# deeplearning-wisc/MCM

Measured on AMD Instinct MI355X. Metric: images/sec MCM-scored (CLIP-B/16, 1000 prompts), higher is better.
Workload: dtype fp16; 1 GPU; MCM scoring, CLIP-ViT-B/16 (12L vision tower, random-init weights), K=1000 prompts pre-encoded, batch 512/GPU, fp32 NCHW pixels resident in HBM -> [B] scores; batch_per_gpu=512, prompts=1000, parallelism=image-sharded x1

## Files before the change

include/mcm.h:

```cpp
#ifndef MCM_H_
#define MCM_H_

#include <stdint.h>

#ifdef __cplusplus
extern "C" {
#endif

#define MCM_ABI_VERSION 5

#define MCM_OK 0
#define MCM_EINVAL (-1)
#define MCM_ENOMEM (-2)
#define MCM_EHIP (-3)
#define MCM_ENOWEIGHT (-4)
#define MCM_ENAME (-5)
#define MCM_ESHAPE (-6)
#define MCM_ERANGE (-7)

#define MCM_PREC_BF16 0
#define MCM_PREC_F32 1
#define MCM_PREC_F16 2

#define MCM_DT_F32 0
// ... 203 lines not shown
int mcm_debug_attention_variant(int32_t variant);
int mcm_debug_attn_spin_budget(int64_t polls);
int mcm_debug_clear_faults(mcm_handle* h);
int mcm_debug_op_attention(mcm_handle* h, int32_t prec, const void* qkv_dev, void* out_dev, int32_t nseq, int32_t seq_len,
                           int32_t heads, int32_t causal, int32_t qrows, int32_t reverse, void* stream);
int mcm_debug_op_attention_split(mcm_handle* h, const void* qkv_dev, void* out_dev, int32_t nseq, int32_t seq_len,
                                 int32_t heads, int32_t qrows, int32_t reverse, void* stream);
int mcm_debug_op_attention_hd(mcm_handle* h, int32_t prec, const void* qkv_dev, void* out_dev, int32_t nseq, int32_t seq_len,
                              int32_t heads, int32_t head_dim, int32_t causal, int32_t qrows, int32_t reverse, void* stream);
int mcm_debug_op_attention_split_hd(mcm_handle* h, const void* qkv_dev, void* out_dev, int32_t nseq, int32_t seq_len,
                                    int32_t heads, int32_t head_dim, int32_t qrows, int32_t reverse, void* stream);
int mcm_debug_vision_front(mcm_handle* h, const void* pixels_dev, int32_t pixel_format, int32_t x2, int32_t B, int32_t stage,
                           int32_t poison, float* resid_out_dev, void* ln_out_dev, void* stream);
int mcm_debug_op_pool_project(mcm_handle* h, const float* x_dev, int64_t x_rows, const int32_t* row_idx_host, int32_t row_stride,
                              int32_t n, int32_t D, const float* gamma_dev, const float* beta_dev, float eps,
                              const float* proj_dev, int32_t P, float* out_dev, int32_t normalize, void* stream);
int mcm_debug_op_text_embed(mcm_handle* h, const int32_t* ids_host, int32_t vocab, const float* tok_dev, const float* pos_dev,
                            float* x_dev, int32_t K, int32_t S, int32_t D, void* stream);
int mcm_debug_gemm_dbg(int32_t bits);
int mcm_debug_qkv_chunks(int32_t n);
int mcm_debug_nsplit(int32_t n);
int mcm_debug_gemm_group_n(int32_t gn);
int mcm_debug_patch_fold(int32_t on);
int mcm_debug_resize_fused_only(int32_t on);
int mcm_debug_persistent_grid(int32_t n);
int mcm_debug_ln_fold(int32_t on);
int mcm_debug_qkv_head_major(int32_t on);
int mcm_debug_ln_tail(int32_t on);
int mcm_debug_ln_cluster(int32_t on);
int mcm_debug_ln_cluster_spin(int32_t polls);
int mcm_debug_ln_row(int32_t on);
int mcm_debug_ln_cluster_deferred(mcm_handle* h, uint64_t* count_host);
int mcm_debug_ln_tail_timeouts(mcm_handle* h, uint64_t* count_host);
#endif

#ifdef __cplusplus
}
#endif
#endif
```

mcm_amd/csrc/attention.hip:

```cpp
#include "common.hpp"

namespace {

__device__ __forceinline__ int ktile_off(int r, int c) {
  const int p = r >> 1;
  return p * 256 + ((((r & 1) << 3) | ((c ^ p) & 7)) << 4);
}

#ifdef MCM_HARNESS
__host__ __device__ constexpr int vt_stride(int LP) {
  return ((LP * 2 - 16 + 255) / 256) * 256 + 16;
}

template <int PREC, int LP, bool CAUSAL>
__global__ __launch_bounds__(256, 2) void attn_bf16_kernel(const uint16_t* __restrict__ qkv,
                                                           uint16_t* __restrict__ out, int L,
                                                           int heads, int qrows, int rev) {
  enter_precision_mode<PREC>();
  extern __shared__ __attribute__((aligned(16))) char smem[];
  constexpr int NT = LP / 16;
  constexpr int NU = LP / 32;
  constexpr int VS = vt_stride(LP);
  constexpr int MAXQB = (LP / 16 + 3) / 4;
  char* Ks = smem;
// ... 1537 lines not shown
  const int nt = (L + 15) / 16;
#ifdef MCM_HARNESS
  if (g_attn_variant == 10 && nseq % 8 == 0) rev |= 2;
  if (g_attn_variant == 11) rev |= 4;
#endif
  bool persistent = nt == 13 && !causal && !hm && qrows == L && (int64_t)nseq * heads >= 16 * (int64_t)device_cu_count();
#ifdef MCM_HARNESS
  if (g_attn_variant == 36) persistent = false;
  if (g_attn_variant == 21) persistent = nt == 13 && !causal && !hm;
#endif
  if (persistent) return launch_ps<PREC, 13, 12, 4>(qkv, out, nseq, L, heads, qrows, s, rev, fault);
#define MCM_TR_EXACT(N, W, O) \
  if (nt == N && !causal) return launch_tr<PREC, N, W, O, false, N - 1>(qkv, out, nseq, L, heads, false, qrows, s, rev, hm)
  MCM_TR_EXACT(4, 4, 3); MCM_TR_EXACT(13, 8, 3); MCM_TR_EXACT(17, 8, 3);
#undef MCM_TR_EXACT
#define MCM_TR(N, W, O) \
  if (nt <= N) return launch_tr<PREC, N, W, O>(qkv, out, nseq, L, heads, causal, qrows, s, rev, hm)
  MCM_TR(1, 4, 3); MCM_TR(2, 4, 3); MCM_TR(3, 4, 3); MCM_TR(4, 4, 3); MCM_TR(5, 4, 3); MCM_TR(6, 4, 3);
  MCM_TR(8, 4, 3); MCM_TR(10, 8, 3); MCM_TR(13, 8, 3); MCM_TR(17, 8, 3); MCM_TR(18, 8, 3);
#undef MCM_TR
  return hipErrorInvalidValue;
}


}

#ifdef MCM_HARNESS
void attention_set_variant(int v) { g_attn_variant = v; }
void attention_set_spin_budget(unsigned int polls) { g_ps_spin_budget = polls; }
#endif

hipError_t launch_attention(int prec, const void* qkv, void* out, int nseq, int L, int heads, int head_dim,
                            bool causal, int qrows, hipStream_t s, bool reverse, int hm, bool split, unsigned int* fault) {
  if (nseq <= 0 || L <= 0 || heads <= 0) return hipErrorInvalidValue;
  if (head_dim != 64 && head_dim != H80) return hipErrorInvalidValue;
  if (qrows <= 0 || qrows > L) qrows = L;
  if (head_dim == H80) {
    if (causal || hm || L > LONG_MAX_L) return hipErrorInvalidValue;
    const int rv = reverse ? 1 : 0;
    if (split) {
      if (prec != MCM_PREC_F16 || (heads * H80) % 64) return hipErrorInvalidValue;
      return launch_hd80<MCM_PREC_F16, true>(qkv, out, nseq, L, heads, qrows, s, rv);
    }
    if (prec == MCM_PREC_F16) return launch_hd80<MCM_PREC_F16, false>(qkv, out, nseq, L, heads, qrows, s, rv);
    if (prec == MCM_PREC_BF16) return launch_hd80<MCM_PREC_BF16, false>(qkv, out, nseq, L, heads, qrows, s, rv);
    if (prec == MCM_PREC_F32) return launch_hd80<MCM_PREC_F32, false>(qkv, out, nseq, L, heads, qrows, s, rv);
    return hipErrorInvalidValue;
// ... 76 lines not shown
```

mcm_amd/csrc/common.hpp:

```cpp
#pragma once
#include <hip/hip_runtime.h>
#include <stdint.h>

#include "../../include/mcm.h"

struct PerDeviceFlag {
  bool done[64] = {};
  static int dev() { int d = 0; return hipGetDevice(&d) == hipSuccess && d >= 0 && d < 64 ? d : -1; }
  bool get() const { const int d = dev(); return d >= 0 && done[d]; }
  void set() { const int d = dev(); if (d >= 0) done[d] = true; }
};

inline int device_cu_count() {
  static int cus[64] = {};
  int dev = 0;
  if (hipGetDevice(&dev) != hipSuccess || dev < 0) return 0;
  if (dev < 64 && cus[dev] > 0) return cus[dev];
  int n = 0;
  if (hipDeviceGetAttribute(&n, hipDeviceAttributeMultiprocessorCount, dev) != hipSuccess) return 0;
  if (dev < 64) cus[dev] = n;
  return n;
}

typedef __attribute__((ext_vector_type(8))) __bf16 bf16x8_t;
// ... 230 lines not shown
hipError_t launch_gemm_row64_ln(int prec, const GemmArgs& a, hipStream_t s, int stages);
hipError_t launch_row64_block_w(const void* w, void* blocked, int N, int K, hipStream_t s);
void gemm_set_group_n(int gn);
void gemm_set_dbg(int d);
void gemm_set_variant(int v);
void attention_set_variant(int v);
void attention_set_spin_budget(unsigned int polls);
#endif

hipError_t launch_layernorm(int prec, const float* x, const float* g, const float* b, void* y,
                            int M, int D, float eps, bool out_f32, hipStream_t s,
                            size_t x_stride = 0, size_t y_stride = 0, bool reverse = false,
                            unsigned int* sat = nullptr, bool split = false);

hipError_t launch_layernorm_pre(int prec, float* x, const float* g0, const float* b0, const float* g1,
                                const float* b1, void* y, int M, int D, float eps, hipStream_t s,
                                bool reverse = false, unsigned int* sat = nullptr, const float* cls = nullptr,
                                const float* pos0 = nullptr, int ntok = 0, bool split = false);

hipError_t launch_attention(int prec, const void* qkv, void* out, int nseq, int L, int heads, int head_dim,
                            bool causal, int qrows, hipStream_t s, bool reverse = false, int hm = 0, bool split = false,
                            unsigned int* fault = nullptr);

hipError_t launch_patchify(int prec, const float* pixels, void* patches, int B, int image,
                           int patch, int kpad, hipStream_t s, bool split = false);
hipError_t launch_patchify_u8(int prec, const uint8_t* pixels, void* patches, int B, int image,
                              int patch, int kpad, const float* mean, const float* stdv,
                              hipStream_t s, bool split = false);
hipError_t launch_bank_reduce(const float* feats, int K, int T, int P, float* bank, hipStream_t s);
hipError_t launch_text_embed(const int32_t* ids, const float* tok, const float* pos, float* x,
                             int K, int S, int D, hipStream_t s);
hipError_t launch_cvt_weight(int prec, const float* src, void* dst, int rows, int cols,
                             int cols_pad, hipStream_t s);
hipError_t launch_cvt_weight_split(int prec, const float* src, void* dst, int rows, int cols,
                                   int cols_pad, hipStream_t s);
hipError_t launch_count_inexact(int prec, const float* src, size_t n, unsigned long long* count, hipStream_t s);

hipError_t launch_pool_project(const float* x, const int32_t* row_idx, int row_stride, int n,
                               int D, const float* g, const float* b, float eps,
                               const float* proj, int P, float* out, hipStream_t s,
                               bool normalize = true);
hipError_t launch_maha_prepare(const float* means, const float* prec, int C, int P, double* w, double* c,
                               hipStream_t s);
hipError_t launch_maha_score(const float* feats, int B, const float* prec, const double* w, const double* c,
                             int C, int P, float* scores, hipStream_t s);
hipError_t launch_maha_fit(const float* feats, int B, int P, const float* shift, double* gram, double* sum,
// ... 44 lines not shown
```

mcm_amd/csrc/embed.hip:

```cpp
#include "common.hpp"

namespace {

template <int OUT, bool X2 = false>
__global__ __launch_bounds__(256) void patchify_kernel(const float* __restrict__ px, void* out,
                                                       int B, int S, int P, int kpad) {
  const int g = S / P, np = g * g, kreal = 3 * P * P;
  const size_t total = (size_t)B * np * kpad;
  for (size_t i = (size_t)blockIdx.x * 256 + threadIdx.x; i < total;
       i += (size_t)gridDim.x * 256) {
    const int k = (int)(i % kpad);
    const size_t m = i / kpad;
    float v = 0.f;
    if (k < kreal) {
      const int b = (int)(m / np), p = (int)(m % np);
      const int gy = p / g, gx = p % g;
      const int c = k / (P * P), rem = k % (P * P), py = rem / P, pxx = rem % P;
      v = px[(((size_t)b * 3 + c) * S + gy * P + py) * S + gx * P + pxx];
    }
    if constexpr (X2) {
      const _Float16 hi = (_Float16)v;
      _Float16* dst = (_Float16*)out + m * 2 * kpad + split_col(k);
      dst[0] = hi;
      dst[64] = (_Float16)(v - (float)hi);
// ... 172 lines not shown
  for (int i = 0; i < NWP; ++i) tot += red[i];
  const float mean = tot / (float)D;
  const float c = tid < D ? xv - mean : 0.f;
  float cw = 0.f;
  float q;
  if constexpr (WIDE) {
    if (t2 < D) cw = xw - mean;
    q = wave_sum(fmaf(cw, cw, c * c));
  } else {
    q = wave_sum(c * c);
  }
  if (lane == 0) red[NWP + wave] = q;
  __syncthreads();
  tot = 0.f;
#pragma unroll
  for (int i = 0; i < NWP; ++i) tot += red[NWP + i];
  const float rstd = 1.0f / sqrtf(tot / (float)D + eps);
  if (tid < D) y[tid] = c * rstd * g[tid] + b[tid];
  if constexpr (WIDE) {
    if (t2 < D) y[t2] = cw * rstd * g[t2] + b[t2];
  }
  __syncthreads();
  float sq = 0.f;
  for (int p = wave; p < P; p += NWP) {
    const float* w = proj + (size_t)p * D;
    float a = 0.f;
    for (int d = lane * 4; d < D; d += 256) {
      const float4 wv = *(const float4*)(w + d);
      a = fmaf(wv.x, y[d], a);
      a = fmaf(wv.y, y[d + 1], a);
      a = fmaf(wv.z, y[d + 2], a);
      a = fmaf(wv.w, y[d + 3], a);
    }
    a = wave_sum(a);
    if (lane == 0) {
      o[p] = a;
      sq += a * a;
    }
  }
  __syncthreads();
  if (lane == 0) red[wave] = sq;
  __syncthreads();
  tot = 0.f;
#pragma unroll
  for (int i = 0; i < NWP; ++i) tot += red[i];
  const float rn = normalize ? 1.0f / sqrtf(tot) : 1.0f;
  for (int p = tid; p < P; p += NWP * 64) out[(size_t)n * P + p] = o[p] * rn;
}

inline int grid_for(size_t total) {
  size_t g = (total + 255) / 256;
  return (int)(g > 4096 ? 4096 : (g ? g : 1));
}

}

hipError_t launch_patchify(int prec, const float* pixels, void* patches, int B, int image,
                           int patch, int kpad, hipStream_t s, bool split) {
  const int g = image / patch;
  if (split) {
// ... 93 lines not shown
```

mcm_amd/csrc/mcm_api.hip:

```cpp
#include <algorithm>
#include <map>
#include <string>
#include <vector>

#include <math.h>
#include <stdlib.h>
#include <string.h>

#include "common.hpp"

namespace {

thread_local std::string g_create_err;

struct Param {
  std::vector<int64_t> shape;
  int64_t numel = 0;
  float* dev = nullptr;
  bool set = false;
};

struct LayerW {
  void *wqkv = nullptr, *wo = nullptr, *w1 = nullptr, *w2 = nullptr;
  float *bqkv = nullptr;
  const float *bo, *b1, *b2, *ln1w, *ln1b, *ln2w, *ln2b;
};

struct Tower {
  int D = 0, heads = 0, layers = 0, ff = 0;
  int prec = MCM_PREC_BF16;
  std::vector<LayerW> L;
  bool split = false;
  int act = MCM_ACT_QUICK_GELU;
};

struct EvPair {
  hipEvent_t a, b;
  int kc, kc2;
};

struct HandleCore {
  mcm_config cfg;
  std::map<std::string, Param> params;
  bool finalized = false;
  Tower vis, txt;
  void* wpatch = nullptr;
  uint64_t w_inexact = 0;
  int kpad = 0, np = 0, ntok = 0;
  float* x = nullptr;
  void *ln = nullptr, *qkv = nullptr, *att = nullptr, *hbuf = nullptr, *patches = nullptr;
  float* feat = nullptr;
  int32_t *ids_dev = nullptr, *rowidx_dev = nullptr;
  int32_t *ids_pin = nullptr, *rowidx_pin = nullptr;
  static constexpr int PREP_RING = 4;
  PrepImage *prep_pin = nullptr, *prep_dev = nullptr;
  int32_t* prep_coef = nullptr;
// ... 98 lines not shown
  }
  ~Scope() {
    if (ev) (void)hipEventRecord(ev->b, s);
  }
};

bool next_dir(HandleCore* h) {
  h->flip = !h->flip;
  return h->flip;
}
int64_t padded_rows(const HandleCore* h, int M) {
  const int64_t mp = ((int64_t)M + 255) / 256 * 256;
  return mp <= h->max_rows ? mp : M;
}

}

#if defined(MCM_HARNESS) || defined(MCM_LN_FOLD) || defined(MCM_LN_TAIL)
#define MCM_API_ARMS 1
#include "mcm_api_arms.hpp"
#else
struct mcm_handle : HandleCore {};
namespace {
constexpr int g_patch_fold = 1, g_resize_fused_only = 0;
struct Arms {
  template <class... A> Arms(A&&...) {}
  template <class... A> void consumer(A&&...) {}
  template <class... A> static constexpr bool qkv_attention(A&&...) { return false; }
  template <class... A> static constexpr bool resid_ln(A&&...) { return false; }
  template <class... A> static constexpr bool column_blocks(A&&...) { return false; }
  template <class... A> static constexpr bool skip_layernorm(A&&...) { return false; }
  template <class... A> static constexpr int create(A&&...) { return MCM_OK; }
  template <class... A> static constexpr int build_layer(A&&...) { return MCM_OK; }
};
}
#endif

namespace {

hipError_t gemm(mcm_handle* h, hipStream_t s, int prec, int epi, const GemmArgs& a_in) {
  hipError_t e = hipSuccess;
  if (Arms::column_blocks(h, s, prec, epi, a_in, e)) return e;
  GemmArgs a = a_in;
  a.rev = next_dir(h) ? 1 : 0;
  a.sat = h->sat_on ? h->sat_dev : nullptr;
  int shape = -1;
  if (a.M > 4096)
// ... 41 lines not shown
  const int es = prec_esize(P);
  const int ks = t.split ? 1 : 0;
  const int xs = x2 ? 1 : 0;
  const int hd = D / t.heads;
  const bool erf = t.act == MCM_ACT_GELU;
  const int epi_store = x2 ? EPI_STORE_X2 : EPI_STORE;
  const int epi_act = erf ? (x2 ? EPI_GELU_ERF_X2 : EPI_GELU_ERF) : (x2 ? EPI_GELU_X2 : EPI_GELU);
  const size_t wrow = (size_t)D * es * (t.split ? 2 : 1);
  Arms arms(h, s, t, nseq, L, pooled_row0, x2);
  int rc = MCM_OK;
  bool ln1_done = ln1_of_layer0_done;
  for (int l = 0; l < t.layers; ++l) {
    const LayerW& w = t.L[l];
    const bool cls = pooled_row0 && l == t.layers - 1 && L > 1;
    if (!ln1_done) HIP_TRY(h, lnorm(h, s, P, h->x, w.ln1w, w.ln1b, h->ln, M, D, false, x2));
    if (!cls) {
      GemmArgs a{};
      a.x = h->ln; a.w = w.wqkv; a.bias = w.bqkv; a.out = h->qkv;
      a.M = M; a.N = 3 * D; a.K = D; a.ldx = D; a.ldo = 3 * D; a.ksplit = ks; a.xsplit = xs;
      arms.consumer(a, l, false);
      if (!arms.qkv_attention(a, epi_store, causal, rc)) {
        HIP_TRY(h, gemm(h, s, P, epi_store, a));
        HIP_TRY(h, attn(h, s, P, nseq, L, t.heads, hd, causal, 0, 0, 0, x2));
      }
    } else {
      GemmArgs kv{};
      kv.x = h->ln; kv.w = (const char*)w.wqkv + (size_t)D * wrow; kv.bias = w.bqkv + D;
      kv.out = (char*)h->qkv + (size_t)D * es * (1 + xs);
      kv.M = M; kv.N = 2 * D; kv.K = D; kv.ldx = D; kv.ldo = 3 * D; kv.ksplit = ks; kv.xsplit = xs;
      HIP_TRY(h, gemm(h, s, P, epi_store, kv));
      GemmArgs q{};
      q.x = h->ln; q.w = w.wqkv; q.bias = w.bqkv; q.out = h->qkv;
      q.M = nseq; q.N = D; q.K = D; q.ldx = L * D; q.ldo = L * 3 * D; q.ksplit = ks; q.xsplit = xs;
      HIP_TRY(h, gemm(h, s, P, epi_store, q));
      HIP_TRY(h, attn(h, s, P, nseq, L, t.heads, hd, causal, 1, 0, 0, x2));
    }
    if (rc) return rc;
    const int Mr = cls ? nseq : M;
    const int rs = cls ? L * D : D;
    GemmArgs o{};
    o.x = h->att; o.w = w.wo; o.bias = w.bo; o.resid = h->x;
    o.M = Mr; o.N = D; o.K = D; o.ldx = rs; o.ldo = rs; o.ksplit = ks; o.xsplit = xs;
    if (cls || !arms.resid_ln(o, l, false, w.ln2w, w.ln2b, rc)) {
      HIP_TRY(h, gemm(h, s, P, EPI_RESID, o));
      if (!cls) HIP_TRY(h, lnorm(h, s, P, h->x, w.ln2w, w.ln2b, h->ln, M, D, false, x2));
      else HIP_TRY(h, lnorm_strided(h, s, P, h->x, w.ln2w, w.ln2b, h->ln, Mr, D, (size_t)rs, (size_t)D * (1 + xs), x2));
// ... 273 lines not shown
  if (c.precision != MCM_PREC_F32) {
    unsigned long long* cnt = nullptr;
    HIP_TRY(h, hipMalloc((void**)&cnt, sizeof(*cnt)));
    hipError_t e = hipMemset(cnt, 0, sizeof(*cnt));
    for (auto& kv : h->params) {
      const std::string& n = kv.first;
      const bool gemm_w = n.rfind("vision_model.", 0) == 0 && kv.second.shape.size() >= 2 &&
                          (n.find("_proj.weight") != std::string::npos || n.find(".mlp.fc") != std::string::npos ||
                           n.find("patch_embedding.weight") != std::string::npos);
      if (gemm_w && e == hipSuccess)
        e = launch_count_inexact(c.precision, kv.second.dev, (size_t)kv.second.numel, cnt, nullptr);
    }
    unsigned long long v = 0;
    if (e == hipSuccess) e = hipMemcpy(&v, cnt, sizeof(v), hipMemcpyDeviceToHost);
    (void)hipFree(cnt);
    if (e != hipSuccess) return fail(h, MCM_EHIP, std::string("counting inexact weights: ") + hipGetErrorString(e));
    h->w_inexact = v;
  }
  h->vis.split = c.precision != MCM_PREC_F32 &&
                 (c.weight_operands == MCM_WEIGHTS_SPLIT || (c.weight_operands == MCM_WEIGHTS_AUTO && h->w_inexact > 0));
  int rc;
  if ((rc = build_tower(h, h->vis, "vision_model", nullptr))) return rc;
  if ((rc = build_tower(h, h->txt, "text_model", nullptr))) return rc;
  const float* wp = W(h, "vision_model.embeddings.patch_embedding.weight");
  const int kreal = 3 * c.patch_size * c.patch_size;
  if (h->vis.split) HIP_TRY(h, launch_cvt_weight_split(c.precision, wp, h->wpatch, c.v_width, kreal, h->kpad, nullptr));
  else HIP_TRY(h, launch_cvt_weight(c.precision, wp, h->wpatch, c.v_width, kreal, h->kpad, nullptr));
  HIP_TRY(h, hipDeviceSynchronize());
  h->finalized = true;
  return MCM_OK;
}

int mcm_weights_operand_exact(mcm_handle* h, uint64_t* inexact_host, int32_t* split_host) {
  int rc = check_ready(h);
  if (rc) return rc;
  if (inexact_host) *inexact_host = h->w_inexact;
  if (split_host) *split_host = h->vis.split ? 1 : 0;
  return MCM_OK;
}

}

namespace {
const float kClipMean[3] = {0.48145466f, 0.4578275f, 0.40821073f};
const float kClipStd[3] = {0.26862954f, 0.26130258f, 0.27577711f};

// ... 800 lines not shown
  for (int x = 0; x < 8; ++x) {
    unsigned int v = 0;
    HIP_TRY(h, hipMemcpy(&v, h->ln_state + (size_t)x * h->ln_rs + 2 * h->ln_cap8 + 3, sizeof(v), hipMemcpyDeviceToHost));
    *count_host += v;
  }
  return MCM_OK;
}
int mcm_debug_ln_tail_timeouts(mcm_handle* h, uint64_t* count_host) {
  if (!h || !count_host) return MCM_EINVAL;
  *count_host = 0;
  if (!h->ln_state) return MCM_OK;
  HIP_TRY(h, hipDeviceSynchronize());
  for (int x = 0; x < 8; ++x) {
    unsigned int v = 0;
    HIP_TRY(h, hipMemcpy(&v, h->ln_state + (size_t)x * h->ln_rs + h->ln_cap8 + 2, sizeof(v), hipMemcpyDeviceToHost));
    *count_host += v;
  }
  return MCM_OK;
}
int mcm_debug_qkv_head_major(int32_t on) {
  g_qkv_head_major = on ? 1 : 0;
  return MCM_OK;
}
int mcm_debug_patch_fold(int32_t on) {
  g_patch_fold = on ? 1 : 0;
  return MCM_OK;
}
int mcm_debug_persistent_grid(int32_t n) {
  if (n < 0 || n % 8 != 0) return MCM_EINVAL;
  gemm_set_persistent_grid(n);
  return MCM_OK;
}
int mcm_debug_resize_fused_only(int32_t on) {
  g_resize_fused_only = on ? 1 : 0;
  return MCM_OK;
}
int mcm_debug_gemm_group_n(int32_t gn) {
  if (gn < 0 || gn > 64) return MCM_EINVAL;
  gemm_set_group_n(gn);
  return MCM_OK;
}
int mcm_debug_nsplit(int32_t n) {
  if (n < 1 || n > 4) return MCM_EINVAL;
  g_nsplit = n;
  return MCM_OK;
}
// ... 16 lines not shown
```

mcm_amd/csrc/mcm_api_arms.hpp:

```cpp
#pragma once

namespace {
struct ArmLayerW {
  float *cqkv = nullptr, *bqkvf = nullptr, *c1 = nullptr, *b1f = nullptr;
  void *wo_blk = nullptr, *w2_blk = nullptr;
};
}

struct mcm_handle : HandleCore {
  std::vector<ArmLayerW> lw;
  float2 *fold_part = nullptr, *fold_rs = nullptr;
  unsigned int* ln_state = nullptr;
  int ln_rs = 0, ln_cap8 = 0;
};

namespace {

hipError_t gemm(mcm_handle* h, hipStream_t s, int prec, int epi, const GemmArgs& a_in);
hipError_t attn(mcm_handle* h, hipStream_t s, int prec, int nseq, int L, int heads, int hd, bool causal, int qrows, int seq0, int hm,
                bool split);

#ifdef MCM_HARNESS
int g_patch_fold = 1;
int g_resize_fused_only = 0;
int g_nsplit = 1;
int g_qkv_head_major = 0;
int g_qkv_chunks = 1;
int g_ln_fold = 0;
int g_ln_tail = 0;
int g_ln_cluster = 0;
int g_ln_row = 0;
int g_lnc_spin = -1;
#else
constexpr int g_patch_fold = 1, g_resize_fused_only = 0, g_qkv_head_major = 0, g_qkv_chunks = 1;
constexpr int g_ln_cluster = 0, g_lnc_spin = -1, g_ln_row = 0;
#ifdef MCM_LN_FOLD
constexpr int g_ln_fold = 1, g_ln_tail = 0;
#else
constexpr int g_ln_fold = 0, g_ln_tail = 1;
#endif
#endif

__global__ void xcc_probe_kernel(unsigned int* out) {
  if (threadIdx.x == 0) {
    unsigned int id;
    asm volatile("s_getreg_b32 %0, hwreg(HW_REG_XCC_ID)" : "=s"(id));
    out[blockIdx.x] = id & 0xfu;
  }
}
bool xcd_round_robin(mcm_handle* h, int grid) {
  if (grid < 8 || grid % 8 || grid > 1024) return false;
  unsigned int* dev = nullptr;
  if (hipMalloc((void**)&dev, (size_t)grid * sizeof(unsigned int)) != hipSuccess) return false;
  std::vector<unsigned int> ids((size_t)grid, 0xffu);
  bool ok = true;
  for (int rep = 0; rep < 3 && ok; ++rep) {
    hipLaunchKernelGGL(xcc_probe_kernel, dim3(grid), dim3(512), 0, 0, dev);
// ... 209 lines not shown
```

mcm_amd/csrc/score.hip:

```cpp
#include "common.hpp"

namespace {

__device__ __forceinline__ double wave_sum_d(double v) {
#pragma unroll
  for (int o = 32; o > 0; o >>= 1) v += __shfl_xor(v, o, 64);
  return v;
}

constexpr int NWV = 16;

__device__ __forceinline__ double block_sum_d(double v, double* red, int lane, int wave) {
  v = wave_sum_d(v);
  __syncthreads();
  if (lane == 0) red[wave] = v;
  __syncthreads();
  double t = 0.0;
#pragma unroll
  for (int i = 0; i < NWV; ++i) t += red[i];
  return t;
}

__device__ __forceinline__ void pair_better(float& v, int& i, float ov, int oi) {
  if (oi >= 0 && (i < 0 || ov > v || (ov == v && oi < i))) {
    v = ov;
    i = oi;
  }
}

template <bool TOPK>
__global__ __launch_bounds__(NWV * 64) void score_kernel(const float* __restrict__ img,
                                                    const float* __restrict__ text, int K, int P,
                                                    float T, int kind, float* __restrict__ scores,
                                                    int topk, int* __restrict__ idx,
                                                    float* __restrict__ prob) {
  extern __shared__ __attribute__((aligned(16))) char smem[];
  float* f = (float*)smem;
  float* sim = f + P;
  __shared__ double red[NWV];
  __shared__ float redf[NWV];
  const int b = blockIdx.x, tid = threadIdx.x, lane = tid & 63, wave = tid >> 6;
  for (int d = tid; d < P; d += NWV * 64) f[d] = img[(size_t)b * P + d];
  __syncthreads();
  for (int k = wave; k < K; k += NWV) {
    const float* t = text + (size_t)k * P;
    float a = 0.f;
    for (int d = lane * 4; d < P; d += 256) {
      const float4 tv = *(const float4*)(t + d);
      const float4 fv = *(const float4*)(f + d);
      a = fmaf(tv.x, fv.x, a);
      a = fmaf(tv.y, fv.y, a);
      a = fmaf(tv.z, fv.z, a);
      a = fmaf(tv.w, fv.w, a);
    }
    a = wave_sum(a);
    if (lane == 0) sim[k] = a;
  }
  __syncthreads();
  float m = -INFINITY;
  for (int k = tid; k < K; k += NWV * 64) m = fmaxf(m, sim[k]);
  m = wave_max(m);
  if (lane == 0) redf[wave] = m;
  __syncthreads();
  m = redf[0];
#pragma unroll
  for (int i = 1; i < NWV; ++i) m = fmaxf(m, redf[i]);
  float selv = 0.f;
  int seli = -1;
  if constexpr (TOPK) {
    __shared__ float stv[2][NWV];
    __shared__ int sti[2][NWV];
    float pv = INFINITY;
    int pi = -1;
    for (int r = 0; r < topk; ++r) {
      float bv = 0.f;
      int bi = -1;
      for (int k = tid; k < K; k += NWV * 64) {
        const float v = sim[k];
        if ((v < pv || (v == pv && k > pi)) && (bi < 0 || v > bv)) {
// ... 283 lines not shown
```

mcm_amd/engine.py:

```python
from __future__ import annotations

import ctypes
import os
from typing import Dict, Optional

import numpy as np

from .config import (ABI_VERSION, CConfig, ClipGeometry, DT_BF16, DT_F16, DT_F32, PREC_BF16, PREC_F16, PREC_F32,
                     SCORE_KINDS, WEIGHT_OPERANDS, geometry)

_HERE = os.path.dirname(os.path.abspath(__file__))
LIB_PATH = os.path.join(_HERE, "libmcm_hip.so")
HARNESS_LIB_PATH = os.path.join(_HERE, "libmcm_hip_harness.so")
KERNEL_CLASSES = ["patchify", "gemm", "layernorm", "attention", "pool_project", "score", "embed",
                  "gemm_qkv", "gemm_outproj", "gemm_fc1", "gemm_fc2"]

TOPK_MAX = 8

_libs = {}


class NativeLibraryMissing(RuntimeError):
    pass

# ... 42 lines not shown
    L.mcm_kernel_faults.argtypes = [vp]
    L.mcm_kernel_faults.restype = i32
    L.mcm_encode_image_x2.argtypes = [vp, vp, i32, i32, i32, vp, vp]
    L.mcm_score_x2.argtypes = [vp, vp, i32, i32, vp, i32, f32, i32, vp, vp]
    if harness:
        L.mcm_debug_gemm_variant.argtypes = [i32]
        L.mcm_debug_op_act.argtypes = [vp, i32, vp, vp, ctypes.c_int64, vp]
        L.mcm_debug_attention_variant.argtypes = [i32]
        L.mcm_debug_attn_spin_budget.argtypes = [ctypes.c_int64]
        L.mcm_debug_clear_faults.argtypes = [vp]
        L.mcm_debug_qkv_chunks.argtypes = [i32]
        L.mcm_debug_ln_fold.argtypes = [i32]
        L.mcm_debug_qkv_head_major.argtypes = [i32]
        L.mcm_debug_ln_tail.argtypes = [i32]
        L.mcm_debug_ln_cluster.argtypes = [i32]
        L.mcm_debug_ln_cluster_spin.argtypes = [i32]
        L.mcm_debug_ln_row.argtypes = [i32]
        L.mcm_debug_ln_cluster_deferred.argtypes = [vp, vp]
        L.mcm_debug_ln_tail_timeouts.argtypes = [vp, vp]
        L.mcm_debug_gemm_dbg.argtypes = [i32]
        L.mcm_debug_nsplit.argtypes = [i32]
        L.mcm_debug_gemm_group_n.argtypes = [i32]
        L.mcm_debug_patch_fold.argtypes = [i32]
        L.mcm_debug_resize_fused_only.argtypes = [i32]
        L.mcm_debug_persistent_grid.argtypes = [i32]
        L.mcm_debug_op_attention.argtypes = [vp, i32, vp, vp, i32, i32, i32, i32, i32, i32, vp]
        L.mcm_debug_op_attention_split.argtypes = [vp, vp, vp, i32, i32, i32, i32, i32, vp]
        L.mcm_debug_op_attention_hd.argtypes = [vp, i32, vp, vp, i32, i32, i32, i32, i32, i32, i32, vp]
        L.mcm_debug_op_attention_split_hd.argtypes = [vp, vp, vp, i32, i32, i32, i32, i32, i32, vp]
        L.mcm_debug_vision_front.argtypes = [vp, vp, i32, i32, i32, i32, i32, vp, vp, vp]
        L.mcm_debug_op_pool_project.argtypes = [vp, vp, ctypes.c_int64, vp, i32, i32, i32, vp, vp, f32, vp, i32, vp, i32, vp]
        L.mcm_debug_op_text_embed.argtypes = [vp, vp, i32, vp, vp, vp, i32, i32, i32, vp]
    L.mcm_encode_image_u8.argtypes = [vp, vp, i32, vp, vp]
    L.mcm_score_u8.argtypes = [vp, vp, i32, vp, i32, f32, i32, vp, vp]
    L.mcm_reduce_bank.argtypes = [vp, vp, i32, i32, vp, vp]
    L.mcm_resize_crop_u8.argtypes = [vp, ctypes.POINTER(vp), ctypes.POINTER(i32), ctypes.POINTER(i32), i32, vp, vp]
    L.mcm_jpeg_reconstruct.argtypes = [vp, vp, vp, vp, i32, vp, ctypes.POINTER(ctypes.c_int64), vp]
    L.mcm_jpeg_entropy_decode.argtypes = [ctypes.POINTER(ctypes.c_char_p), i32, vp, ctypes.c_int64, vp, vp, i32,
                                          ctypes.POINTER(ctypes.c_int64)]
    L.mcm_pack_u8.argtypes = [ctypes.POINTER(vp), ctypes.POINTER(ctypes.c_int64), ctypes.POINTER(ctypes.c_int64), i32, vp,
                              ctypes.c_int64, i32]
    L.mcm_tokenizer_create.argtypes = [ctypes.c_char_p, ctypes.c_char_p, ctypes.POINTER(vp)]
    L.mcm_tokenizer_destroy.argtypes = [vp]
    L.mcm_tokenizer_destroy.restype = None
    L.mcm_tokenizer_last_error.argtypes = [vp]
    L.mcm_tokenizer_last_error.restype = ctypes.c_char_p
# ... 28 lines not shown
    "mcm_op_attention", "mcm_encode_image_u8", "mcm_score_u8",
    "mcm_reduce_bank", "mcm_measures", "mcm_resize_crop_u8", "mcm_tokenizer_create",
    "mcm_tokenizer_destroy", "mcm_tokenizer_last_error", "mcm_tokenizer_vocab_size", "mcm_tokenizer_encode",
    "mcm_encode_image_raw", "mcm_maha_prepare", "mcm_maha_score_features",
    "mcm_encode_image_ex", "mcm_encode_text_ex", "mcm_score_histogram",
    "mcm_saturation_check", "mcm_saturation_count",
    "mcm_weights_operand_exact", "mcm_op_linear_ex", "mcm_op_split_weight", "mcm_pack_u8",
    "mcm_jpeg_entropy_decode", "mcm_jpeg_reconstruct",
    "mcm_x2_max_batch", "mcm_encode_image_x2", "mcm_score_x2", "mcm_op_layernorm_split", "mcm_op_attention_split",
    "mcm_kernel_faults",
    "mcm_score_features_topk", "mcm_score_topk",
    "mcm_maha_fit_accumulate",
    "mcm_knn_workspace_bytes", "mcm_knn_score_features",
    "mcm_neglabel_workspace_bytes", "mcm_neglabel_score_features",
]
HARNESS_ONLY_SYMBOLS = ["mcm_debug_gemm_variant", "mcm_debug_attention_variant", "mcm_debug_qkv_chunks",
                        "mcm_debug_gemm_dbg", "mcm_debug_ln_fold", "mcm_debug_qkv_head_major",
                        "mcm_debug_ln_tail", "mcm_debug_ln_tail_timeouts", "mcm_debug_nsplit",
                        "mcm_debug_gemm_group_n", "mcm_debug_patch_fold", "mcm_debug_resize_fused_only",
                        "mcm_debug_persistent_grid", "mcm_debug_op_attention", "mcm_debug_attn_spin_budget",
                        "mcm_debug_clear_faults", "mcm_debug_ln_cluster", "mcm_debug_ln_cluster_spin",
                        "mcm_debug_ln_cluster_deferred", "mcm_debug_ln_row", "mcm_debug_op_attention_split",
                        "mcm_debug_vision_front", "mcm_debug_op_pool_project", "mcm_debug_op_text_embed",
                        "mcm_debug_op_act", "mcm_debug_op_attention_hd", "mcm_debug_op_attention_split_hd"]


def _stream_ptr():
    import torch

    return ctypes.c_void_p(torch.cuda.current_stream().cuda_stream)


class NativeCLIP:

    def __init__(self, geo: ClipGeometry | str, state_dict: Dict[str, np.ndarray], *,
                 device: int = 0, precision: str = "fp16", max_batch: int = 512,
                 max_prompt_tokens: int = 1024 * 77, synthetic_weights: Optional[bool] = None,
                 harness: bool = False, weight_operands: str = "auto", x2_max_batch: Optional[int] = None):
        import torch

        if not torch.cuda.is_available():
            raise RuntimeError("NativeCLIP needs a HIP device (no CPU fallback)")
        self.geo = geometry(geo) if isinstance(geo, str) else geo
        self.device = torch.device("cuda", device)
        self.x2_default = precision == "fp16x2"
        self.precision = {"bf16": PREC_BF16, "fp32": PREC_F32, "f32": PREC_F32, "fp16": PREC_F16,
                          "f16": PREC_F16, "fp16x2": PREC_F16}[precision]
# ... 468 lines not shown
```

Measured before the change: 26230 images/sec.

## Fold K projection into CLS query for last-layer CLS-only attention

In the last vision layer only the CLS row's output is needed. Instead of projecting K and V for every token, the change projects only Q for the CLS row and multiplies it by a per-head K weight block precomputed at load time. The resulting vectors score the LayerNorm'd tokens directly, the attention-weighted LN rows are accumulated, and the V projection plus bias is applied once per head afterwards. This removes the full-sequence K/V GEMM in the final layer, at the cost of an extra heads*D*D weight buffer and new custom kernels. Separately, the image projection and text-similarity dot-product loops now compute four rows per wave to expose more memory-level parallelism.

```diff
diff --git a/include/mcm.h b/include/mcm.h
--- a/include/mcm.h
+++ b/include/mcm.h
@@ -249,6 +249,10 @@
 int mcm_debug_nsplit(int32_t n);
 int mcm_debug_gemm_group_n(int32_t gn);
 int mcm_debug_patch_fold(int32_t on);
+int mcm_debug_cls_fold(int32_t on);
+int mcm_debug_op_cls_fold(mcm_handle* h, int32_t prec, const void* ln_dev, const void* q_dev, const void* wk_dev, const void* wv_dev,
+                          const float* bv_dev, void* out_dev, int32_t nseq, int32_t seq_len, int32_t seq_rows, int32_t heads,
+                          void* stream);
 int mcm_debug_resize_fused_only(int32_t on);
 int mcm_debug_persistent_grid(int32_t n);
 int mcm_debug_ln_fold(int32_t on);
diff --git a/mcm_amd/csrc/attention.hip b/mcm_amd/csrc/attention.hip
--- a/mcm_amd/csrc/attention.hip
+++ b/mcm_amd/csrc/attention.hip
@@ -1583,7 +1583,219 @@
   return hipErrorInvalidValue;
 }
 
-
+constexpr int CF_NW = 8;
+constexpr int CF_MAXKB = 8;
+constexpr int CF_TLS = CF_MAXKB * 16 + 4;
+
+template <int PREC>
+__device__ __forceinline__ void unpack2(uint32_t v, float& lo, float& hi) {
+  if constexpr (PREC == MCM_PREC_F16) {
+    typedef _Float16 h2_t __attribute__((ext_vector_type(2)));
+    const h2_t h = __builtin_bit_cast(h2_t, v);
+    lo = (float)h[0];
+    hi = (float)h[1];
+  } else {
+    lo = __builtin_bit_cast(float, v << 16);
+    hi = __builtin_bit_cast(float, v & 0xffff0000u);
+  }
+}
+
+template <int PREC, int MAXKB, int OCC>
+__global__ __launch_bounds__(CF_NW * 64, OCC) void attn_cls_fold_kernel(const uint16_t* __restrict__ ln, const uint16_t* __restrict__ u,
+                                                                   uint16_t* __restrict__ z, int L, int heads, int D,
+                                                                   int seq_rows, unsigned int* sat) {
+  __shared__ float spart[2][CF_NW][16][16];
+  __shared__ __attribute__((aligned(16))) uint16_t tl[CF_NW][16][CF_TLS];
+  enter_precision_mode<PREC>();
+  const int n = blockIdx.x, lane = threadIdx.x & 63, wave = threadIdx.x >> 6, r16 = lane & 15, g = lane >> 4;
+  const int cw = D / CF_NW, nkb = cw / 16, c0 = wave * cw + 4 * g;
+  constexpr float SC = 0.125f * 1.4426950408889634f;
+  const uint2 zero2 = make_uint2(0u, 0u);
+  float amax = 0.f;
+
+  uint2 ureg[MAXKB];
+  {
+    const uint16_t* ur = u + ((size_t)n * heads + (r16 < heads ? r16 : 0)) * D + c0;
+#pragma unroll
+    for (int kb = 0; kb < MAXKB; ++kb)
+      ureg[kb] = (kb < nkb && r16 < heads) ? *(const uint2*)(ur + kb * 16) : zero2;
+  }
+  const uint16_t* lnn = ln + (size_t)n * seq_rows * D + c0;
+  uint2 cur[MAXKB], nxt[MAXKB];
+  auto load = [&](int t0, uint2* dst) {
+    const int tok = t0 + r16;
+    const uint16_t* p = lnn + (size_t)(tok < L ? tok : 0) * D;
+#pragma unroll
+    for (int kb = 0; kb < MAXKB; ++kb) dst[kb] = (kb < nkb && tok < L) ? *(const uint2*)(p + kb * 16) : zero2;
+  };
+  f32x4_t zacc[MAXKB];
+#pragma unroll
+  for (int kb = 0; kb < MAXKB; ++kb) {
+    zacc[kb] = f32x4_t{0.f, 0.f, 0.f, 0.f};
+    nxt[kb] = zero2;
+  }
+  float m_run = -INFINITY, l_run = 0.f;
+  load(0, cur);
+  const int nch = (L + 15) / 16;
+  for (int c = 0; c < nch; ++c) {
+    if (c + 1 < nch) load((c + 1) * 16, nxt);
+    f32x4_t s = {0.f, 0.f, 0.f, 0.f};
+#pragma unroll
+    for (int kb = 0; kb < MAXKB; ++kb)
+      if (kb < nkb) s = mfma16<PREC>(make_uint4(cur[kb].x, cur[kb].y, 0u, 0u), make_uint4(ureg[kb].x, ureg[kb].y, 0u, 0u), s);
+    asm volatile("" ::: "memory");
+#pragma unroll
+    for (int r = 0; r < 4; ++r) spart[c & 1][wave][4 * g + r][r16] = s[r];
+#pragma unroll
+    for (int kb = 0; kb < MAXKB; ++kb)
+      if (kb < nkb) *(uint2*)&tl[wave][r16][kb * 16 + 4 * g] = cur[kb];
+    __syncthreads();
+    float sv[4];
+#pragma unroll
+    for (int r = 0; r < 4; ++r) {
+      float a = 0.f;
+#pragma unroll
+      for (int w = 0; w < CF_NW; ++w) a += spart[c & 1][w][4 * g + r][r16];
+      sv[r] = c * 16 + 4 * g + r < L ? a : -INFINITY;
+    }
+    float cm = fmaxf(fmaxf(sv[0], sv[1]), fmaxf(sv[2], sv[3]));
+    cm = fmaxf(cm, __shfl_xor(cm, 16, 64));
+    cm = fmaxf(cm, __shfl_xor(cm, 32, 64));
+    const float mn = fmaxf(m_run, cm);
+    const float alpha = __builtin_amdgcn_exp2f((m_run - mn) * SC);
+    const float msc = mn * SC;
+    float e[4];
+#pragma unroll
+    for (int r = 0; r < 4; ++r) e[r] = __builtin_amdgcn_exp2f(fmaf(sv[r], SC, -msc));
+    const uint32_t p01 = pack2<PREC>(e[0], e[1]), p23 = pack2<PREC>(e[2], e[3]);
+    sat_track<PREC>(amax, e[0], e[1]);
+    sat_track<PREC>(amax, e[2], e[3]);
+    float q0, q1, q2, q3;
+    unpack2<PREC>(p01, q0, q1);
+    unpack2<PREC>(p23, q2, q3);
+    float ps = (q0 + q1) + (q2 + q3);
+    ps += __shfl_xor(ps, 16, 64);
+    ps += __shfl_xor(ps, 32, 64);
+    l_run = fmaf(l_run, alpha, ps);
+    m_run = mn;
+    float ar[4];
+#pragma unroll
+    for (int r = 0; r < 4; ++r) ar[r] = __shfl(alpha, 4 * g + r, 64);
+    const uint4 pa = make_uint4(p01, p23, 0u, 0u);
+#pragma unroll
+    for (int kb = 0; kb < MAXKB; ++kb)
+      if (kb < nkb) {
+        const uint16_t* t = &tl[wave][4 * g][kb * 16 + r16];
+        const uint32_t b01 = (uint32_t)t[0] | ((uint32_t)t[CF_TLS] << 16), b23 = (uint32_t)t[2 * CF_TLS] | ((uint32_t)t[3 * CF_TLS] << 16);
+#pragma unroll
+        for (int r = 0; r < 4; ++r) zacc[kb][r] *= ar[r];
+        zacc[kb] = mfma16<PREC>(pa, make_uint4(b01, b23, 0u, 0u), zacc[kb]);
+      }
+#pragma unroll
+    for (int kb = 0; kb < MAXKB; ++kb) cur[kb] = nxt[kb];
+  }
+  float inv[4];
+#pragma unroll
+  for (int r = 0; r < 4; ++r) inv[r] = 1.0f / __shfl(l_run, 4 * g + r, 64);
+#pragma unroll
+  for (int kb = 0; kb < MAXKB; ++kb)
+    if (kb < nkb) {
+#pragma unroll
+      for (int r = 0; r < 4; ++r) {
+        const int head = 4 * g + r;
+        const float v = zacc[kb][r] * inv[r];
+        sat_track<PREC>(amax, v, 0.f);
+        if (head < heads) z[((size_t)n * heads + head) * D + wave * cw + kb * 16 + r16] = (uint16_t)(pack2<PREC>(v, 0.f) & 0xffffu);
+      }
+    }
+  sat_report<PREC>(amax, sat);
+}
+
+template <int PREC>
+__global__ __launch_bounds__(64) void cls_vproj_kernel(const uint16_t* __restrict__ z, const uint16_t* __restrict__ wv,
+                                                       const float* __restrict__ bv, uint16_t* __restrict__ out, int nseq,
+                                                       int heads, int D, size_t out_rows_stride, unsigned int* sat) {
+  enter_precision_mode<PREC>();
+  const int h = blockIdx.x, i0 = blockIdx.y * 16, lane = threadIdx.x, r16 = lane & 15, g = lane >> 4;
+  const int img = i0 + r16 < nseq ? i0 + r16 : nseq - 1;
+  const uint16_t* zr = z + ((size_t)img * heads + h) * D + 8 * g;
+  const uint16_t* wr = wv + (size_t)(h * 64 + r16) * D + 8 * g;
+  f32x4_t acc[4];
+#pragma unroll
+  for (int cb = 0; cb < 4; ++cb) acc[cb] = f32x4_t{0.f, 0.f, 0.f, 0.f};
+  for (int k = 0; k < D; k += 32) {
+    const uint4 a = *(const uint4*)(zr + k);
+#pragma unroll
+    for (int cb = 0; cb < 4; ++cb) acc[cb] = mfma16<PREC>(a, *(const uint4*)(wr + (size_t)cb * 16 * D + k), acc[cb]);
+  }
+  float amax = 0.f;
+#pragma unroll
+  for (int cb = 0; cb < 4; ++cb) {
+    const int col = h * 64 + cb * 16 + r16;
+    const float b = bv[col];
+#pragma unroll
+    for (int r = 0; r < 4; ++r) {
+      const int im = i0 + 4 * g + r;
+      const float v = acc[cb][r] + b;
+      sat_track<PREC>(amax, v, 0.f);
+      if (im < nseq) out[(size_t)im * out_rows_stride + col] = (uint16_t)(pack2<PREC>(v, 0.f) & 0xffffu);
+    }
+  }
+  sat_report<PREC>(amax, sat);
+}
+
+__global__ __launch_bounds__(256) void cls_fold_wk_kernel(const uint16_t* __restrict__ wk, uint16_t* __restrict__ out, int heads, int D) {
+  const size_t total = (size_t)heads * D * D;
+  for (size_t i = (size_t)blockIdx.x * 256 + threadIdx.x; i < total; i += (size_t)gridDim.x * 256) {
+    const int j = (int)(i % D);
+    const size_t row = i / D;
+    const int h = (int)(row / D), n = (int)(row % D);
+    out[i] = (j >> 6) == h ? wk[(size_t)j * D + n] : (uint16_t)0;
+  }
+}
+
+}
+
+bool cls_fold_shape_ok(int prec, int heads, int D) {
+  return prec != MCM_PREC_F32 && heads >= 1 && heads <= 16 && D == heads * 64 && D % (CF_NW * 16) == 0 && D <= CF_NW * CF_MAXKB * 16;
+}
+
+hipError_t launch_cls_fold_wk(const void* wk, void* out, int heads, int D, hipStream_t s) {
+  if (!wk || !out || heads < 1 || D != heads * 64) return hipErrorInvalidValue;
+  const size_t blocks = ((size_t)heads * D * D + 255) / 256;
+  hipLaunchKernelGGL(cls_fold_wk_kernel, dim3((unsigned)(blocks < 4096 ? blocks : 4096)), dim3(256), 0, s, (const uint16_t*)wk,
+                     (uint16_t*)out, heads, D);
+  return hipGetLastError();
+}
+
+hipError_t launch_cls_fold_attention(int prec, const void* ln, const void* u, void* z, int nseq, int L, int seq_rows, int heads,
+                                     int D, hipStream_t s, unsigned int* sat) {
+  if (!cls_fold_shape_ok(prec, heads, D) || nseq <= 0 || L <= 0 || seq_rows < L || !ln || !u || !z) return hipErrorInvalidValue;
+#define MCM_CLS_FOLD(P, KB, OCC)                                                                                              \
+  hipLaunchKernelGGL((attn_cls_fold_kernel<P, KB, OCC>), dim3(nseq), dim3(CF_NW * 64), 0, s, (const uint16_t*)ln, (const uint16_t*)u, \
+                     (uint16_t*)z, L, heads, D, seq_rows, sat)
+  if (D <= CF_NW * 6 * 16) {
+    if (prec == MCM_PREC_F16) MCM_CLS_FOLD(MCM_PREC_F16, 6, 4);
+    else MCM_CLS_FOLD(MCM_PREC_BF16, 6, 4);
+  } else {
+    if (prec == MCM_PREC_F16) MCM_CLS_FOLD(MCM_PREC_F16, 8, 3);
+    else MCM_CLS_FOLD(MCM_PREC_BF16, 8, 3);
+  }
+#undef MCM_CLS_FOLD
+  return hipGetLastError();
+}
+
+hipError_t launch_cls_vproj(int prec, const void* z, const void* wv, const float* bv, void* out, int nseq, int heads, int D,
+                            size_t out_rows_stride, hipStream_t s, unsigned int* sat) {
+  if (!cls_fold_shape_ok(prec, heads, D) || nseq <= 0 || !z || !wv || !bv || !out) return hipErrorInvalidValue;
+  const dim3 grid(heads, (nseq + 15) / 16);
+  if (prec == MCM_PREC_F16)
+    hipLaunchKernelGGL(cls_vproj_kernel<MCM_PREC_F16>, grid, dim3(64), 0, s, (const uint16_t*)z, (const uint16_t*)wv, bv, (uint16_t*)out,
+                       nseq, heads, D, out_rows_stride, sat);
+  else
+    hipLaunchKernelGGL(cls_vproj_kernel<MCM_PREC_BF16>, grid, dim3(64), 0, s, (const uint16_t*)z, (const uint16_t*)wv, bv, (uint16_t*)out,
+                       nseq, heads, D, out_rows_stride, sat);
+  return hipGetLastError();
 }
 
 #ifdef MCM_HARNESS
diff --git a/mcm_amd/csrc/common.hpp b/mcm_amd/csrc/common.hpp
--- a/mcm_amd/csrc/common.hpp
+++ b/mcm_amd/csrc/common.hpp
@@ -276,6 +276,13 @@
                             bool causal, int qrows, hipStream_t s, bool reverse = false, int hm = 0, bool split = false,
                             unsigned int* fault = nullptr);
 
+bool cls_fold_shape_ok(int prec, int heads, int D);
+hipError_t launch_cls_fold_wk(const void* wk, void* out, int heads, int D, hipStream_t s);
+hipError_t launch_cls_fold_attention(int prec, const void* ln, const void* u, void* z, int nseq, int L, int seq_rows, int heads,
+                                     int D, hipStream_t s, unsigned int* sat = nullptr);
+hipError_t launch_cls_vproj(int prec, const void* z, const void* wv, const float* bv, void* out, int nseq, int heads, int D,
+                            size_t out_rows_stride, hipStream_t s, unsigned int* sat = nullptr);
+
 hipError_t launch_patchify(int prec, const float* pixels, void* patches, int B, int image,
                            int patch, int kpad, hipStream_t s, bool split = false);
 hipError_t launch_patchify_u8(int prec, const uint8_t* pixels, void* patches, int B, int image,
diff --git a/mcm_amd/csrc/embed.hip b/mcm_amd/csrc/embed.hip
--- a/mcm_amd/csrc/embed.hip
+++ b/mcm_amd/csrc/embed.hip
@@ -218,20 +218,36 @@
   }
   __syncthreads();
   float sq = 0.f;
-  for (int p = wave; p < P; p += NWP) {
-    const float* w = proj + (size_t)p * D;
-    float a = 0.f;
+  for (int p0 = wave; p0 < P; p0 += 4 * NWP) {
+    const float* w[4];
+    float a[4];
+#pragma unroll
+    for (int c = 0; c < 4; ++c) {
+      const int p = p0 + c * NWP;
+      w[c] = proj + (size_t)(p < P ? p : p0) * D;
+      a[c] = 0.f;
+    }
     for (int d = lane * 4; d < D; d += 256) {
-      const float4 wv = *(const float4*)(w + d);
-      a = fmaf(wv.x, y[d], a);
-      a = fmaf(wv.y, y[d + 1], a);
-      a = fmaf(wv.z, y[d + 2], a);
-      a = fmaf(wv.w, y[d + 3], a);
-    }
-    a = wave_sum(a);
+      float4 wv[4];
+#pragma unroll
+      for (int c = 0; c < 4; ++c) wv[c] = *(const float4*)(w[c] + d);
+#pragma unroll
+      for (int c = 0; c < 4; ++c) {
+        a[c] = fmaf(wv[c].x, y[d], a[c]);
+        a[c] = fmaf(wv[c].y, y[d + 1], a[c]);
+        a[c] = fmaf(wv[c].z, y[d + 2], a[c]);
+        a[c] = fmaf(wv[c].w, y[d + 3], a[c]);
+      }
+    }
+#pragma unroll
+    for (int c = 0; c < 4; ++c) a[c] = wave_sum(a[c]);
     if (lane == 0) {
-      o[p] = a;
-      sq += a * a;
+#pragma unroll
+      for (int c = 0; c < 4; ++c)
+        if (p0 + c * NWP < P) {
+          o[p0 + c * NWP] = a[c];
+          sq += a[c] * a[c];
+        }
     }
   }
   __syncthreads();
diff --git a/mcm_amd/csrc/mcm_api.hip b/mcm_amd/csrc/mcm_api.hip
--- a/mcm_amd/csrc/mcm_api.hip
+++ b/mcm_amd/csrc/mcm_api.hip
@@ -32,6 +32,7 @@
   std::vector<LayerW> L;
   bool split = false;
   int act = MCM_ACT_QUICK_GELU;
+  void* wkf = nullptr;
 };
 
 struct EvPair {
@@ -176,7 +177,7 @@
 #else
 struct mcm_handle : HandleCore {};
 namespace {
-constexpr int g_patch_fold = 1, g_resize_fused_only = 0;
+constexpr int g_patch_fold = 1, g_resize_fused_only = 0, g_cls_fold = 1;
 struct Arms {
   template <class... A> Arms(A&&...) {}
   template <class... A> void consumer(A&&...) {}
@@ -264,6 +265,26 @@
       if (!arms.qkv_attention(a, epi_store, causal, rc)) {
         HIP_TRY(h, gemm(h, s, P, epi_store, a));
         HIP_TRY(h, attn(h, s, P, nseq, L, t.heads, hd, causal, 0, 0, 0, x2));
+      }
+    } else if (g_cls_fold && t.wkf && !causal && !x2 && (size_t)2 * nseq * t.heads * D * es <= h->hbuf_bytes) {
+      GemmArgs q{};
+      q.x = h->ln; q.w = w.wqkv; q.bias = w.bqkv; q.out = h->qkv;
+      q.M = nseq; q.N = D; q.K = D; q.ldx = L * D; q.ldo = L * 3 * D;
+      HIP_TRY(h, gemm(h, s, P, EPI_STORE, q));
+      GemmArgs uf{};
+      uf.x = h->qkv; uf.w = t.wkf; uf.out = h->hbuf;
+      uf.M = nseq; uf.N = t.heads * D; uf.K = D; uf.ldx = L * 3 * D; uf.ldo = t.heads * D;
+      HIP_TRY(h, gemm(h, s, P, EPI_STORE, uf));
+      void* zf = (char*)h->hbuf + (size_t)nseq * t.heads * D * es;
+      unsigned int* sat = h->sat_on ? h->sat_dev : nullptr;
+      {
+        Scope sc(h, s, MCM_KC_ATTENTION, 4.0 * nseq * t.heads * (double)L * D);
+        HIP_TRY(h, launch_cls_fold_attention(P, h->ln, h->hbuf, zf, nseq, L, L, t.heads, D, s, sat));
+      }
+      {
+        Scope sc(h, s, MCM_KC_ATTENTION, 2.0 * nseq * (double)D * D);
+        HIP_TRY(h, launch_cls_vproj(P, zf, (const char*)w.wqkv + (size_t)2 * D * wrow, w.bqkv + 2 * D, h->att, nseq, t.heads, D,
+                                    (size_t)L * D, s, sat));
       }
     } else {
       GemmArgs kv{};
@@ -583,6 +604,12 @@
   int rc;
   if ((rc = build_tower(h, h->vis, "vision_model", nullptr))) return rc;
   if ((rc = build_tower(h, h->txt, "text_model", nullptr))) return rc;
+  if (!h->vis.split && h->vis.layers > 0 && cls_fold_shape_ok(c.precision, h->vis.heads, h->vis.D)) {
+    const int D = h->vis.D;
+    const size_t es = prec_esize(c.precision);
+    if ((rc = dev_alloc(h, &h->vis.wkf, (size_t)h->vis.heads * D * D * es))) return rc;
+    HIP_TRY(h, launch_cls_fold_wk((const char*)h->vis.L.back().wqkv + (size_t)D * D * es, h->vis.wkf, h->vis.heads, D, nullptr));
+  }
   const float* wp = W(h, "vision_model.embeddings.patch_embedding.weight");
   const int kreal = 3 * c.patch_size * c.patch_size;
   if (h->vis.split) HIP_TRY(h, launch_cvt_weight_split(c.precision, wp, h->wpatch, c.v_width, kreal, h->kpad, nullptr));
@@ -1429,6 +1456,37 @@
   g_qkv_head_major = on ? 1 : 0;
   return MCM_OK;
 }
+int mcm_debug_cls_fold(int32_t on) {
+  g_cls_fold = on ? 1 : 0;
+  return MCM_OK;
+}
+int mcm_debug_op_cls_fold(mcm_handle* h, int32_t prec, const void* ln_dev, const void* q_dev, const void* wk_dev, const void* wv_dev,
+                          const float* bv_dev, void* out_dev, int32_t nseq, int32_t seq_len, int32_t seq_rows, int32_t heads,
+                          void* stream) {
+  if (!h) return MCM_EINVAL;
+  const int D = heads * 64;
+  if (!cls_fold_shape_ok(prec, heads, D) || nseq < 1 || seq_len < 1 || seq_rows < seq_len || !ln_dev || !q_dev || !wk_dev || !wv_dev ||
+      !bv_dev || !out_dev)
+    return fail(h, MCM_EINVAL, "cls_fold: a 16-bit mode, heads <= 16 with D = 64 heads a multiple of 128, device pointers");
+  hipStream_t s = (hipStream_t)stream;
+  const size_t es = prec_esize(prec);
+  char* work = nullptr;
+  const size_t wkb = (size_t)heads * D * D * es, ub = (size_t)nseq * heads * D * es;
+  HIP_TRY(h, hipMalloc((void**)&work, wkb + 2 * ub));
+  hipError_t e = launch_cls_fold_wk(wk_dev, work, heads, D, s);
+  GemmArgs uf{};
+  uf.x = q_dev; uf.w = work; uf.out = work + wkb;
+  uf.M = nseq; uf.N = heads * D; uf.K = D; uf.ldx = D; uf.ldo = heads * D;
+  if (e == hipSuccess) e = gemm(h, s, prec, EPI_STORE, uf);
+  unsigned int* sat = h->sat_on ? h->sat_dev : nullptr;
+  if (e == hipSuccess) e = launch_cls_fold_attention(prec, ln_dev, work + wkb, work + wkb + ub, nseq, seq_len, seq_rows, heads, D, s, sat);
+  if (e == hipSuccess) e = launch_cls_vproj(prec, work + wkb + ub, wv_dev, bv_dev, out_dev, nseq, heads, D, (size_t)D, s, sat);
+  if (e == hipSuccess) e = hipStreamSynchronize(s);
+  (void)hipFree(work);
+  HIP_TRY(h, e);
+  return MCM_OK;
+}
+
 int mcm_debug_patch_fold(int32_t on) {
   g_patch_fold = on ? 1 : 0;
   return MCM_OK;
diff --git a/mcm_amd/csrc/mcm_api_arms.hpp b/mcm_amd/csrc/mcm_api_arms.hpp
--- a/mcm_amd/csrc/mcm_api_arms.hpp
+++ b/mcm_amd/csrc/mcm_api_arms.hpp
@@ -22,6 +22,7 @@
 
 #ifdef MCM_HARNESS
 int g_patch_fold = 1;
+int g_cls_fold = 1;
 int g_resize_fused_only = 0;
 int g_nsplit = 1;
 int g_qkv_head_major = 0;
@@ -32,7 +33,7 @@
 int g_ln_row = 0;
 int g_lnc_spin = -1;
 #else
-constexpr int g_patch_fold = 1, g_resize_fused_only = 0, g_qkv_head_major = 0, g_qkv_chunks = 1;
+constexpr int g_patch_fold = 1, g_cls_fold = 1, g_resize_fused_only = 0, g_qkv_head_major = 0, g_qkv_chunks = 1;
 constexpr int g_ln_cluster = 0, g_lnc_spin = -1, g_ln_row = 0;
 #ifdef MCM_LN_FOLD
 constexpr int g_ln_fold = 1, g_ln_tail = 0;
diff --git a/mcm_amd/csrc/score.hip b/mcm_amd/csrc/score.hip
--- a/mcm_amd/csrc/score.hip
+++ b/mcm_amd/csrc/score.hip
@@ -42,19 +42,35 @@
   const int b = blockIdx.x, tid = threadIdx.x, lane = tid & 63, wave = tid >> 6;
   for (int d = tid; d < P; d += NWV * 64) f[d] = img[(size_t)b * P + d];
   __syncthreads();
-  for (int k = wave; k < K; k += NWV) {
-    const float* t = text + (size_t)k * P;
-    float a = 0.f;
+  for (int k0 = wave; k0 < K; k0 += 4 * NWV) {
+    const float* t[4];
+    float a[4];
+#pragma unroll
+    for (int c = 0; c < 4; ++c) {
+      const int k = k0 + c * NWV;
+      t[c] = text + (size_t)(k < K ? k : k0) * P;
+      a[c] = 0.f;
+    }
     for (int d = lane * 4; d < P; d += 256) {
-      const float4 tv = *(const float4*)(t + d);
       const float4 fv = *(const float4*)(f + d);
-      a = fmaf(tv.x, fv.x, a);
-      a = fmaf(tv.y, fv.y, a);
-      a = fmaf(tv.z, fv.z, a);
-      a = fmaf(tv.w, fv.w, a);
-    }
-    a = wave_sum(a);
-    if (lane == 0) sim[k] = a;
+      float4 tv[4];
+#pragma unroll
+      for (int c = 0; c < 4; ++c) tv[c] = *(const float4*)(t[c] + d);
+#pragma unroll
+      for (int c = 0; c < 4; ++c) {
+        a[c] = fmaf(tv[c].x, fv.x, a[c]);
+        a[c] = fmaf(tv[c].y, fv.y, a[c]);
+        a[c] = fmaf(tv[c].z, fv.z, a[c]);
+        a[c] = fmaf(tv[c].w, fv.w, a[c]);
+      }
+    }
+#pragma unroll
+    for (int c = 0; c < 4; ++c) a[c] = wave_sum(a[c]);
+    if (lane == 0) {
+#pragma unroll
+      for (int c = 0; c < 4; ++c)
+        if (k0 + c * NWV < K) sim[k0 + c * NWV] = a[c];
+    }
   }
   __syncthreads();
   float m = -INFINITY;
diff --git a/mcm_amd/engine.py b/mcm_amd/engine.py
--- a/mcm_amd/engine.py
+++ b/mcm_amd/engine.py
@@ -88,6 +88,8 @@
         L.mcm_debug_nsplit.argtypes = [i32]
         L.mcm_debug_gemm_group_n.argtypes = [i32]
         L.mcm_debug_patch_fold.argtypes = [i32]
+        L.mcm_debug_cls_fold.argtypes = [i32]
+        L.mcm_debug_op_cls_fold.argtypes = [vp, i32, vp, vp, vp, vp, vp, vp, i32, i32, i32, i32, vp]
         L.mcm_debug_resize_fused_only.argtypes = [i32]
         L.mcm_debug_persistent_grid.argtypes = [i32]
         L.mcm_debug_op_attention.argtypes = [vp, i32, vp, vp, i32, i32, i32, i32, i32, i32, vp]
@@ -162,7 +164,8 @@
                         "mcm_debug_clear_faults", "mcm_debug_ln_cluster", "mcm_debug_ln_cluster_spin",
                         "mcm_debug_ln_cluster_deferred", "mcm_debug_ln_row", "mcm_debug_op_attention_split",
                         "mcm_debug_vision_front", "mcm_debug_op_pool_project", "mcm_debug_op_text_embed",
-                        "mcm_debug_op_act", "mcm_debug_op_attention_hd", "mcm_debug_op_attention_split_hd"]
+                        "mcm_debug_op_act", "mcm_debug_op_attention_hd", "mcm_debug_op_attention_split_hd",
+                        "mcm_debug_cls_fold", "mcm_debug_op_cls_fold"]
 
 
 def _stream_ptr():
```

Result: no change. 26490 images/sec (median of 6 runs) (+1.0%).
